# KLab/YAIK

Measured on AMD Instinct MI355X. Metric: Mpix/s tile encode (alpha reject + 7 gradient passes + 8x8 range quant), 8K RGBA, higher is better.
Workload: dtype u8/int32 (+f32 mode-selection sums)

## Files before the change

yaik_amd/csrc/yk_api.hip:

```cpp
#include "yk_common.h"
#ifdef YK_TEST_HOOKS
#include "../../include/yaik_hip_test.h"
#endif
#include <cstdio>
#include <cstring>
#include <utility>
#include <vector>

int yk_fail(yk_ctx* c, int code, const char* what, hipError_t e) {
    if (c && c->err.empty()) {
        c->err = what ? what : "error";
        if (e != hipSuccess) { c->err += ": "; c->err += hipGetErrorString(e); }
    }
    return code;
}

int yk_refuse(yk_ctx* c, int code, const char* what) {
    if (c) c->err = what ? what : "error";
    return code;
}

void yk_rebase(yk_ctx* c, int f) {
    const YkFrameStrides& fs = c->fs; auto& B = c->B;
    c->curFrame = f;
    for (int i = 0; i < 4; i++) c->plane[i] = B.plane[i] ? B.plane[i] + (size_t)f * fs.plane : nullptr;
    c->keep = B.keep + (size_t)f * fs.keep; c->bounds = B.bounds + (size_t)f * 16;
    for (int i = 0; i < 7; i++) c->bitmap[i] = B.bitmap[i] + (size_t)f * fs.bitmap[i];
    c->coverage = B.coverage + (size_t)f * fs.coverage; c->tileDef = B.tileDef + (size_t)f * fs.tileDef;
    c->tileCount = B.tileCount + (size_t)f * fs.tileCount; c->slots = B.slots + (size_t)f * fs.slots;
    c->blockSums = B.blockSums + (size_t)f * fs.blockN; c->blockCnt = B.blockCnt + (size_t)f * fs.blockN;
    c->totals = B.totals + (size_t)f * 8; c->defsOut = B.defsOut + (size_t)f * fs.defsOut; c->nibOut = B.nibOut + (size_t)f * fs.nibOut;
}

static void yk_free_image(yk_ctx* c) {
    auto F = [](auto*& p) { if (p) { (void)hipFree((void*)p); p = nullptr; } };
    auto& B = c->B;
    F(B.keep); F(B.bounds); F(c->alphaUnitBox); F(c->alphaArrive);
    F(B.small);
    for (int i = 0; i < 7; i++) B.bitmap[i] = nullptr;
    B.coverage = nullptr; B.bm0b = nullptr; B.tileInfo = nullptr; B.runSums = nullptr;
    F(B.tileDef); F(B.tileCount); F(B.slots);
    for (int i = 0; i < 3; i++) F(c->dst[i]);
    F(B.blockSums); F(B.blockCnt); F(B.totals); F(c->exportSizes); F(B.defsOut); F(B.nibOut);
    c->keep = nullptr; c->bounds = nullptr; for (int i = 0; i < 7; i++) c->bitmap[i] = nullptr;
    c->coverage = nullptr; c->tileDef = nullptr; c->tileCount = nullptr; c->slots = nullptr;
    c->blockSums = nullptr; c->blockCnt = nullptr; c->totals = nullptr; c->defsOut = nullptr; c->nibOut = nullptr;
    F(c->latticeOwner); F(c->cornerStream); F(c->cornerScratch); F(c->cornerEdgeIdx);
    F(c->preview); F(c->covCh); F(c->mapped3); F(c->ppBitmap); F(c->ppStream); F(c->ppScratch); c->ppBitmapBytes = c->ppBitmapCap = 0; c->ppStreamCap = c->ppStreamBytes = 0; c->ppScratchElems = 0;
    F(c->r1Slots); F(c->r1Params); F(c->r1Cnt); F(c->r1Pix); F(c->r1Type); c->r1Ready = false;
    F(c->pixCache); c->pixCacheValid = false;
    if (c->frameGraph) { (void)hipGraphExecDestroy(c->frameGraph); c->frameGraph = nullptr; }
    c->encoded = false; c->alphaDone = false; c->alphaFinished = false; c->cornersReady = false; c->ppActive = false; c->ppLastBit = 0; c->previewFresh = false;
}

static int yk_alloc_image(yk_ctx* c) {
    const size_t F = (size_t)c->nFrames;
    const size_t T8 = (size_t)c->tilesW * c->tilesH, MT = (size_t)c->mtW * c->mtH;
    auto& B = c->B; YkFrameStrides& fs = c->fs;
    auto up = [](size_t n, size_t a) { return (n + a - 1) / a * a; };
    fs.keep = up(MT + 4, 16);
    YK_HIP(c, hipMalloc(&B.keep, fs.keep * F + 16));
    YK_HIP(c, hipMalloc(&B.bounds, 16 * sizeof(int32_t) * F));
    {
        const size_t nUnits = (size_t)((c->fullW / 4 + 63) / 64) * c->mtH, nGroups = (nUnits + 63) / 64;
        YK_HIP(c, hipMalloc(&c->alphaUnitBox, (nUnits + nGroups) * F * 4 * sizeof(int) + 16));
        YK_HIP(c, hipMalloc(&c->alphaArrive, (nGroups + 1) * F * sizeof(uint32_t) + 16));
        YK_HIP(c, hipMemset(c->alphaArrive, 0, (nGroups + 1) * F * sizeof(uint32_t) + 16));
    }
    static const int sh[7][2] = { {4,4},{4,3},{3,4},{3,3},{3,2},{2,3},{2,2} };
    size_t cur = 0, oBm[7], oBm0b, oCov, oInfo, oRun;
    auto place = [&](size_t bytesPerFrame) { const size_t o = cur; cur = up(cur + bytesPerFrame * F + 16, 256); return o; };
    for (int i = 0; i < 7; i++) {
        const int bx = (sh[i][0] == 2) ? 32 : 64, by = (sh[i][1] == 2) ? 32 : 64;
        const size_t bits = (size_t)((c->fullW + bx - 1) / bx) * ((c->h + by - 1) / by) * ((bx >> sh[i][0]) * (by >> sh[i][1]));
        c->bitmapBytes[i] = bits >> 3;
        fs.bitmap[i] = up(c->bitmapBytes[i] + 4, 16);
        oBm[i] = place(fs.bitmap[i]);
    }
    const size_t nB64 = (size_t)((c->fullW + 63) / 64) * ((c->h + 63) / 64);
    fs.bm0b = up(nB64 * 4, 16); oBm0b = place(fs.bm0b);
    fs.coverage = up(MT, 8); oCov = place(fs.coverage * sizeof(uint16_t));
    fs.tileInfo = up(T8, 2); oInfo = place(fs.tileInfo * sizeof(uint2));
    fs.runSums = up((T8 + 7) / 8, 4); oRun = place(fs.runSums * sizeof(uint32_t));
    if (cur >= ((size_t)1 << 32)) return yk_fail(c, YK_ERR_BAD_ARG, "image too large for 32-bit offsets into the small-output arena");
    YK_HIP(c, hipMalloc(&B.small, cur));
    YK_HIP(c, hipMemset(B.small, 0, cur));
    for (int i = 0; i < 7; i++) B.bitmap[i] = B.small + oBm[i];
    B.bm0b = B.small + oBm0b; B.coverage = reinterpret_cast<uint16_t*>(B.small + oCov);
    B.tileInfo = reinterpret_cast<uint2*>(B.small + oInfo); B.runSums = reinterpret_cast<uint32_t*>(B.small + oRun);
    fs.tileDef = 3 * T8; fs.tileCount = 3 * T8; fs.slots = 3 * T8 * YK_SLOT;
    YK_HIP(c, hipMalloc(&B.tileDef, fs.tileDef * F * sizeof(uint16_t) + 16));
    YK_HIP(c, hipMalloc(&B.tileCount, fs.tileCount * F + 16));
    YK_HIP(c, hipMalloc(&B.slots, fs.slots * F + 16));
    c->nScanBlocks = (int)((T8 + 1023) / 1024);
    fs.blockN = (size_t)c->nScanBlocks * 2;
    YK_HIP(c, hipMalloc(&B.blockSums, fs.blockN * F * sizeof(uint32_t)));
    YK_HIP(c, hipMalloc(&B.blockCnt, fs.blockN * F * sizeof(uint32_t)));
    YK_HIP(c, hipMemset(B.blockCnt, 0, fs.blockN * F * sizeof(uint32_t)));
    YK_HIP(c, hipMalloc(&B.totals, 8 * sizeof(uint32_t) * F));
    fs.defsOut = 3 * T8;
// ... 75 lines not shown
int yk_create(int device, yk_ctx** out) {
    if (!out) return YK_ERR_BAD_ARG;
    *out = nullptr;
    int n = 0;
    if (hipGetDeviceCount(&n) != hipSuccess || n <= 0) return YK_ERR_NO_DEVICE;
    if (device < 0 || device >= n) return YK_ERR_BAD_ARG;
    if (hipSetDevice(device) != hipSuccess) return YK_ERR_NO_DEVICE;
    yk_ctx* c = new yk_ctx();
    c->device = device;
    if (hipDeviceGetAttribute(&c->numCU, hipDeviceAttributeMultiprocessorCount, device) != hipSuccess || c->numCU <= 0) c->numCU = 256;
    if (hipStreamCreateWithFlags(&c->ownStream, hipStreamNonBlocking) != hipSuccess) { delete c; return YK_ERR_HIP; }
    c->stream = c->ownStream;
    for (int r = 0; r < YK_EV_RING; r++) for (int i = 0; i < 5; i++) if (hipEventCreate(&c->evRing[r][i]) != hipSuccess) { delete c; return YK_ERR_HIP; }
    if (yk_qtab_get(c) != YK_OK) { yk_destroy(c); return YK_ERR_HIP; }
    *out = c;
    return YK_OK;
}

void yk_destroy(yk_ctx* c) {
    if (!c) return;
    (void)hipSetDevice(c->device);
    (void)hipStreamSynchronize(c->stream);
    yk_free_image(c);
    yk_lut_destroy(c);
    yk_lut_dec_destroy(c);
    auto F = [](auto*& p) { if (p) { (void)hipFree((void*)p); p = nullptr; } };
    yk_dec_free(c);
    F(c->ownedPlanes); F(c->pxStage); F(c->dScratch); F(c->dAlpha); F(c->dAvScratch); F(c->avState); F(c->avPay); F(c->av6);
    for (int r = 0; r < YK_EV_RING; r++) for (int i = 0; i < 5; i++) if (c->evRing[r][i]) (void)hipEventDestroy(c->evRing[r][i]);
    for (int st = 0; st < YK_NUM_STAGES; st++) for (int k = 0; k < YK_STAGE_RING; k++) for (int i = 0; i < 2; i++) if (c->stEv[st][k][i]) (void)hipEventDestroy(c->stEv[st][k][i]);
    if (c->frameGraph) (void)hipGraphExecDestroy(c->frameGraph);
    if (c->evHandoff) (void)hipEventDestroy(c->evHandoff);
    if (c->evPixCopy) (void)hipEventDestroy(c->evPixCopy);
    if (c->evFusedAfter) (void)hipEventDestroy(c->evFusedAfter);
    if (c->auxStream) (void)hipStreamDestroy(c->auxStream);
    if (c->ownStream) (void)hipStreamDestroy(c->ownStream);
    delete c;
}

const char* yk_last_error(const yk_ctx* c) { return c ? c->err.c_str() : "null handle"; }

int yk_set_stream(yk_ctx* c, void* s) {
    if (!c) return YK_ERR_BAD_ARG;
    hipStream_t next = s ? (hipStream_t)s : c->ownStream;
    if (next == c->stream) return YK_OK;
    YK_HIP(c, hipSetDevice(c->device));
    if (!c->evHandoff) YK_HIP(c, hipEventCreateWithFlags(&c->evHandoff, hipEventDisableTiming));
    if (hipEventRecord(c->evHandoff, c->stream) == hipSuccess) YK_HIP(c, hipStreamWaitEvent(next, c->evHandoff, 0));
    else (void)hipGetLastError();
    c->stream = next;
    return YK_OK;
}

int yk_synchronize(yk_ctx* c) {
    if (!c) return YK_ERR_BAD_ARG;
    YK_HIP(c, hipSetDevice(c->device));
    YK_HIP(c, hipStreamSynchronize(c->stream));
    return YK_OK;
}

int yk_set_image(yk_ctx* c, int fullW, int fullH, int nPlanes, int y0, int h, int haloRows) {
    if (!c) return YK_ERR_BAD_ARG;
    if (fullW < 8 || fullH < 8 || (fullW & 7) || (fullH & 7) || fullW > 32760 || fullH > 32760) return yk_fail(c, YK_ERR_BAD_ARG, "image size must be a multiple of 8 and fit s16 fields");
    if (nPlanes != 3 && nPlanes != 4) return yk_fail(c, YK_ERR_BAD_ARG, "nPlanes must be 3 or 4");
    if (y0 < 0 || h < 8 || (h & 7) || y0 + h > fullH || (y0 & 63)) return yk_fail(c, YK_ERR_BAD_ARG, "stripe rows must start on a multiple of 64 and lie inside the image");
    if (y0 + h < fullH && ((h & 63) || haloRows != 1)) return yk_fail(c, YK_ERR_BAD_ARG, "inner stripes need h % 64 == 0 and one halo row");
    if (y0 + h == fullH && haloRows != 0) return yk_fail(c, YK_ERR_BAD_ARG, "the last stripe has no halo row");
    YK_HIP(c, hipSetDevice(c->device));
// ... 328 lines not shown
    YK_HIP(c, hipSetDevice(c->device));
    if (wantDst) {
        const size_t n = (size_t)c->fullW * c->h;
        for (int p = 0; p < 3; p++) {
            if (!c->dst[p]) YK_HIP(c, hipMalloc(&c->dst[p], n * sizeof(int32_t)));
            if (c->dstFill == 0 || c->dstFill == -1) YK_HIP(c, hipMemsetAsync(c->dst[p], c->dstFill & 255, n * sizeof(int32_t), c->stream));
            else {
                std::vector<int32_t> f(n, c->dstFill);
                YK_HIP(c, hipMemcpyAsync(c->dst[p], f.data(), n * sizeof(int32_t), hipMemcpyHostToDevice, c->stream));
                YK_HIP(c, hipStreamSynchronize(c->stream));
            }
        }
    }
    hipEvent_t* ev = c->evRing[c->evHead % YK_EV_RING];
    if (!c->evAlphaInCur) { YK_HIP(c, hipEventRecord(ev[0], c->stream)); YK_HIP(c, hipEventRecord(ev[1], c->stream)); }
    if (c->fusedAfter) { YK_HIP(c, hipStreamWaitEvent(c->stream, c->fusedAfter, 0)); c->fusedAfter = nullptr; }
    YK_HIP(c, hipEventRecord(ev[2], c->stream));
    int rc = yk_launch_encode(c, rejectFactor, mode3BitOnly, wantDst); if (rc) return rc;
    YK_HIP(c, hipEventRecord(ev[3], c->stream));
    rc = yk_launch_pack(c); if (rc) return rc;
    YK_HIP(c, hipEventRecord(ev[4], c->stream));
    c->evAlphaInCur = false;
    c->evHead++;
    if (c->evHead - c->evTail > YK_EV_RING) c->evTail = c->evHead - YK_EV_RING;
    c->encoded = true; c->dstValid = wantDst != 0; c->cornersReady = false; c->ppActive = false; c->ppLastBit = 0; c->previewFresh = false; c->nextCornerPass = 0; c->r1Ready = false;
    return YK_OK;
}

int yk_order_fused_after(yk_ctx* c, const yk_ctx* other) {
    if (!c || !other) return YK_ERR_BAD_ARG;
    if (c->device != other->device) return yk_fail(c, YK_ERR_BAD_ARG, "yk_order_fused_after: handles of one device");
    c->fusedAfter = nullptr;
    if (!other->evHead) return YK_OK;
    YK_HIP(c, hipSetDevice(c->device));
    if (!c->auxStream) YK_HIP(c, hipStreamCreateWithFlags(&c->auxStream, hipStreamNonBlocking));
    if (!c->evFusedAfter) YK_HIP(c, hipEventCreateWithFlags(&c->evFusedAfter, hipEventDisableTiming));
    static const int afterPack = getenv("YK_ORDER_AFTER_PACK") ? atoi(getenv("YK_ORDER_AFTER_PACK")) : 0;
    YK_HIP(c, hipStreamWaitEvent(c->auxStream, other->evRing[(other->evHead - 1) % YK_EV_RING][afterPack ? 4 : 3], 0));
    YK_HIP(c, hipEventRecord(c->evFusedAfter, c->auxStream));
    c->fusedAfter = c->evFusedAfter;
    return YK_OK;
}

int yk_encode_batch(yk_ctx* c, int rejectFactor, int mode3BitOnly) {
    if (!c) return YK_ERR_BAD_ARG;
    if (!c->B.plane[0]) return yk_fail(c, YK_ERR_STATE, "bind planes first");
    if (rejectFactor < 0 || rejectFactor > 64) return yk_fail(c, YK_ERR_BAD_ARG, "rejectFactor out of range");
    if (c->y0 != 0 || c->h != c->fullH) return yk_fail(c, YK_ERR_STATE, "batches hold whole images");
    if (c->kernelVersion != 2) return yk_fail(c, YK_ERR_STATE, "batches need kernel version 2");
    if (c->nFrames > 1 && c->fs.plane == 0) return yk_fail(c, YK_ERR_STATE, "yk_bind_device_batch first");
    YK_HIP(c, hipSetDevice(c->device));
    hipEvent_t* ev = c->evRing[c->evHead % YK_EV_RING];
    YK_HIP(c, hipEventRecord(ev[0], c->stream));
    int rc = YK_OK;
    if (c->nPlanes == 4) rc = yk_launch_alpha(c, true);
    if (rc) return rc;
    YK_HIP(c, hipEventRecord(ev[1], c->stream));
    if (c->fusedAfter) { YK_HIP(c, hipStreamWaitEvent(c->stream, c->fusedAfter, 0)); c->fusedAfter = nullptr; }
    YK_HIP(c, hipEventRecord(ev[2], c->stream));
    rc = yk_launch_encode(c, rejectFactor, mode3BitOnly, 0, true); if (rc) return rc;
    YK_HIP(c, hipEventRecord(ev[3], c->stream));
    rc = yk_launch_pack(c, true); if (rc) return rc;
    YK_HIP(c, hipEventRecord(ev[4], c->stream));
    c->evAlphaInCur = false; c->evHead++;
    if (c->evHead - c->evTail > YK_EV_RING) c->evTail = c->evHead - YK_EV_RING;
    c->alphaDone = c->nPlanes == 4; c->alphaFinished = true;
    c->encoded = true; c->dstValid = false; c->cornersReady = false; c->ppActive = false; c->ppLastBit = 0; c->previewFresh = false; c->nextCornerPass = 0; c->r1Ready = false;
    return YK_OK;
}

int yk_encode_frame(yk_ctx* c, int rejectFactor, int mode3BitOnly) {
    if (!c) return YK_ERR_BAD_ARG;
    if (!c->plane[0]) return yk_fail(c, YK_ERR_STATE, "bind planes first");
// ... 239 lines not shown
```

yaik_amd/csrc/yk_common.h:

```cpp
#pragma once
#include <hip/hip_runtime.h>
#include <stdint.h>
#include <stddef.h>
#include <string>
#include "../../include/yaik_hip.h"

#define YK_BLK      64
#define YK_LSTRIDE  68
#define YK_LROWS    65
#define YK_EV_RING  64
#define YK_SLOT     32
#define YK_NUM_STAGES 8
#define YK_STAGE_RING 16

struct YkFrameStrides {
    unsigned long long plane, keep, bitmap[7], coverage, tileDef, tileCount, slots, blockN, defsOut, nibOut;
    unsigned long long bm0b, tileInfo, runSums;
};

struct YkEncodeParams {
    const int32_t* plane[4];
    int strideElems;
    int w, h;
    int hAvail;
// ... 14 lines not shown
    int xBB64, yBB64, xBB32, yBB32;
    int nFrames;
    const uint8_t* qtab;
    uint8_t* small;
    uint32_t oBm[7], oBm0b, oCov, oInfo, oRun;
    uint4* pixCache;
    YkFrameStrides fs;
};

struct yk_ctx {
    int device = -1;
    int numCU = 256;
    const uint8_t* qtab = nullptr;
    hipStream_t ownStream = nullptr;
    hipStream_t stream = nullptr;
    std::string err;
    int fullW = 0, fullH = 0, nPlanes = 0, y0 = 0, h = 0, halo = 0;
    int tilesW = 0, tilesH = 0, mtW = 0, mtH = 0;
    int nFrames = 1, curFrame = 0;
    YkFrameStrides fs = {};
    struct Bases {
        const int32_t* plane[4]; uint8_t* keep; int32_t* bounds; uint8_t* bitmap[7]; uint16_t* coverage; uint16_t* tileDef; uint8_t* tileCount;
        uint8_t* slots; uint32_t* blockSums; uint32_t* blockCnt; uint32_t* totals; uint16_t* defsOut; uint8_t* nibOut;
        uint8_t* small;
        uint8_t* bm0b; uint2* tileInfo; uint32_t* runSums;
    } B = {};
    const int32_t* plane[4] = {nullptr, nullptr, nullptr, nullptr};
    int strideElems = 0;
    int32_t* ownedPlanes = nullptr; size_t ownedPlanesBytes = 0;
    uint8_t* pxStage = nullptr; size_t pxStageBytes = 0;
    hipEvent_t evPixCopy = nullptr;
    uint8_t* keep = nullptr;
    int32_t* bounds = nullptr;
    int* alphaUnitBox = nullptr;
    uint32_t* alphaArrive = nullptr;
    int boundsOff = 8;
    bool alphaDone = false, alphaFinished = false;
    int32_t hostBounds[4] = {0, 0, 0, 0}; int hostDiscard = 1, hostHasChunk = 0;
    uint8_t* bitmap[7] = {}; size_t bitmapBytes[7] = {};
    uint16_t* coverage = nullptr;
    uint16_t* tileDef = nullptr; uint8_t* tileCount = nullptr; uint8_t* slots = nullptr;
    int32_t* dst[3] = {nullptr, nullptr, nullptr}; int32_t dstFill = -1; bool dstValid = false;
    uint32_t* blockSums = nullptr;
    uint32_t* blockCnt = nullptr;
    uint32_t* totals = nullptr;
    unsigned long long* exportSizes = nullptr;
    hipEvent_t evHandoff = nullptr;
    hipEvent_t fusedAfter = nullptr;
    hipEvent_t evFusedAfter = nullptr; hipStream_t auxStream = nullptr;
    uint16_t* defsOut = nullptr;
    uint8_t*  nibOut = nullptr;
    size_t nibStride = 0;
    int nScanBlocks = 0;
    bool encoded = false;
    uint32_t* latticeOwner = nullptr; size_t latticeElems = 0;
    uint8_t* cornerStream = nullptr; size_t cornerCap = 0;
    uint32_t* cornerScratch = nullptr; size_t cornerScratchElems = 0;
    uint32_t* cornerEdgeIdx = nullptr;
    bool cornersReady = false; int nextCornerPass = 0;
    size_t cornerOff[7] = {}, cornerBytes[7] = {};
    const uint32_t* cornerTotalsDev = nullptr; bool cornerTotalsPending = false;
    const uint32_t* r1TotalsDev = nullptr; bool r1TotalsPending = false;
    uint16_t* covCh = nullptr; size_t covChStride = 0;
    uint8_t* mapped3 = nullptr;
    uint32_t* ppBitmap = nullptr; size_t ppBitmapBytes = 0; uint8_t* ppStream = nullptr; size_t ppStreamCap = 0, ppStreamBytes = 0;
    uint32_t* ppScratch = nullptr; size_t ppScratchElems = 0, ppBitmapCap = 0; int ppAccepted = 0; bool ppActive = false;
    int ppLastBit = 0, ppLastSx = 0, ppLastSy = 0;
    int32_t* preview = nullptr; bool previewFresh = false;
    struct YkLutState* lut = nullptr;
    struct YkLutDecState* lutDec = nullptr;
    uint8_t* r1Slots = nullptr; uint8_t* r1Params = nullptr; uint32_t* r1Cnt = nullptr; uint8_t* r1Pix = nullptr; uint8_t* r1Type = nullptr;
    uint32_t r1Tiles = 0, r1PixCount = 0; bool r1Ready = false;
    uint4* pixCache = nullptr; bool pixCacheOn = false, pixCacheValid = false;
    uint32_t r1EndTiles[3] = {}, r1EndPix[3] = {};
    int dw = 0, dh = 0; uint8_t* dPlanes = nullptr; size_t dPlaneSize = 0;
    uint8_t* dMapRGB = nullptr; uint32_t* dLatticeOwner = nullptr; uint8_t* dTile4 = nullptr; size_t dTile4Size = 0;
    uint8_t* dScratch = nullptr; size_t dScratchBytes = 0;
    uint8_t* dLoaded = nullptr;
    bool dSplit = false;
    uint8_t* dAlpha = nullptr; size_t dAlphaBytes = 0; bool dAlphaValid = false;
    uint8_t* dAvScratch = nullptr; size_t dAvScratchBytes = 0;
    int32_t* avState = nullptr; uint8_t* avPay = nullptr; size_t avPayCap = 0;
// ... 44 lines not shown
```

yaik_amd/csrc/yk_stages.hip:

```cpp
#include "yk_common.h"
#ifdef YK_TEST_HOOKS
#include "../../include/yaik_hip_test.h"
#endif
#include "yk_device.h"

typedef int yk_i4 __attribute__((ext_vector_type(4)));
#ifndef YK_ALPHA_INFLIGHT
#define YK_ALPHA_INFLIGHT 8
#endif
#ifndef YK_ALPHA_THREADS
#define YK_ALPHA_THREADS 256
#endif
#define YK_ALPHA_WAVES (YK_ALPHA_THREADS / 64)
#ifndef YK_ALPHA_ROWS
#define YK_ALPHA_ROWS 2
#endif
__global__ __launch_bounds__(YK_ALPHA_THREADS) void yk_alpha_kernel(const int32_t* __restrict__ alpha0, int strideElems, int w, int h, int y0,
                                                       uint8_t* __restrict__ keep0, int mtW, int mtH, int32_t* __restrict__ bounds,
                                                       int nFrames, unsigned long long planeStride, unsigned long long keepStride,
                                                       int* __restrict__ unitBox0, uint32_t* __restrict__ arrive0) {
    __shared__ int s_box[YK_ALPHA_WAVES][4];
    const int lane = threadIdx.x & 63, wv = threadIdx.x >> 6;
    const int vecPerRow = w >> 2;
    const int nSeg = (vecPerRow + YK_ALPHA_THREADS - 1) / YK_ALPHA_THREADS;
    const int nRowUnits = (mtH + YK_ALPHA_ROWS - 1) / YK_ALPHA_ROWS;
    const int nUnits = nSeg * nRowUnits, nGroups = (nUnits + 63) >> 6;
    for (long long uu = blockIdx.x; uu < (long long)nUnits * nFrames; uu += gridDim.x) {
        const int f = (int)(uu / nUnits), u = (int)(uu - (long long)f * nUnits);
        const int32_t* alpha = alpha0 + (size_t)f * planeStride;
        uint8_t* keep = keep0 + (size_t)f * keepStride;
        int* unitBox = unitBox0 + (size_t)f * (nUnits + nGroups) * 4;
        uint32_t* arrive = arrive0 + (size_t)f * (nGroups + 1);
        const int tyU = u / nSeg, seg = u - tyU * nSeg;
        const int xv = seg * YK_ALPHA_THREADS + (int)threadIdx.x;
        const bool inX = xv < vecPerRow;
        const bool tileLane = (lane & 3) == 0;
        const int tx = xv >> 2;
        int colLo = 0x7FFFFFFF, colHi = -1, rowLo = 0x7FFFFFFF, rowHi = -1;
#pragma unroll
        for (int r = 0; r < YK_ALPHA_ROWS; r++) {
            const int ty = tyU * YK_ALPHA_ROWS + r;
            if (ty >= mtH) break;
            const int32_t* col = alpha + (size_t)(ty * 16) * strideElems + (size_t)xv * 4;
            int nz = 0;
#pragma unroll
            for (int kb = 0; kb < 16 / YK_ALPHA_INFLIGHT; kb++) {
                yk_i4 a[YK_ALPHA_INFLIGHT];
#pragma unroll
                for (int k = 0; k < YK_ALPHA_INFLIGHT; k++) {
                    const int y = ty * 16 + kb * YK_ALPHA_INFLIGHT + k;
                    a[k] = (yk_i4){0, 0, 0, 0};
                    if (inX && y < h) a[k] = __builtin_nontemporal_load(reinterpret_cast<const yk_i4*>(col + (size_t)(kb * YK_ALPHA_INFLIGHT + k) * strideElems));
                }
#pragma unroll
                for (int k = 0; k < YK_ALPHA_INFLIGHT; k++) nz |= a[k].x | a[k].y | a[k].z | a[k].w;
            }
            const unsigned long long b = __ballot(nz != 0);
            const bool kept = ((b >> (lane & ~3)) & 0xFULL) != 0;
            if (tileLane && tx < mtW) keep[(size_t)ty * mtW + tx] = kept ? 1 : 0;
            const unsigned long long kb64 = __ballot(tileLane && kept && tx < mtW);
            if (kb64) {
                const int t0 = seg * (YK_ALPHA_THREADS / 4) + wv * 16;
                colLo = min(colLo, t0 + ((__ffsll((long long)kb64) - 1) >> 2));
                colHi = max(colHi, t0 + ((63 - __clzll((long long)kb64)) >> 2));
                rowLo = min(rowLo, ty); rowHi = max(rowHi, ty);
            }
        }
        if (lane == 0) { s_box[wv][0] = colLo; s_box[wv][1] = colHi; s_box[wv][2] = rowLo; s_box[wv][3] = rowHi; }
        __syncthreads();
        if (wv == 0) {
            unsigned long long* ub = reinterpret_cast<unsigned long long*>(unitBox);
            auto putBox = [&](const int slot, const int bx0, const int by0, const int bx1, const int by1) {
                __hip_atomic_store(&ub[slot * 2], ((unsigned long long)(uint32_t)by0 << 32) | (uint32_t)bx0, __ATOMIC_RELAXED, __HIP_MEMORY_SCOPE_AGENT);
                __hip_atomic_store(&ub[slot * 2 + 1], ((unsigned long long)(uint32_t)by1 << 32) | (uint32_t)bx1, __ATOMIC_RELAXED, __HIP_MEMORY_SCOPE_AGENT);
                __builtin_amdgcn_s_waitcnt(0);
            };
            auto foldBoxes = [&](const int first, const int n, int& x0, int& gy0, int& x1, int& gy1) {
                x0 = 9999999; gy0 = 9999999; x1 = -1; gy1 = -1;
                for (int k = lane; k < n; k += 64) {
                    const unsigned long long a = __hip_atomic_load(&ub[(first + k) * 2], __ATOMIC_RELAXED, __HIP_MEMORY_SCOPE_AGENT);
                    const unsigned long long bb = __hip_atomic_load(&ub[(first + k) * 2 + 1], __ATOMIC_RELAXED, __HIP_MEMORY_SCOPE_AGENT);
                    x0 = min(x0, (int)(uint32_t)a); gy0 = min(gy0, (int)(uint32_t)(a >> 32)); x1 = max(x1, (int)(uint32_t)bb); gy1 = max(gy1, (int)(uint32_t)(bb >> 32));
                }
#pragma unroll
                for (int d = 1; d < 64; d <<= 1) {
                    x0 = min(x0, __shfl_xor(x0, d)); x1 = max(x1, __shfl_xor(x1, d));
                    gy0 = min(gy0, __shfl_xor(gy0, d)); gy1 = max(gy1, __shfl_xor(gy1, d));
                }
            };
            const int g = u >> 6, inGroup = min(64, nUnits - (g << 6));
            uint32_t lastOfGroup = 0;
            if (lane == 0) {
                int lo = s_box[0][0], hi = s_box[0][1], rlo = s_box[0][2], rhi = s_box[0][3];
#pragma unroll
                for (int k = 1; k < YK_ALPHA_WAVES; k++) { lo = min(lo, s_box[k][0]); hi = max(hi, s_box[k][1]); rlo = min(rlo, s_box[k][2]); rhi = max(rhi, s_box[k][3]); }
                const bool any = hi >= 0;
                putBox(u, any ? lo * 16 : 9999999, any ? y0 + rlo * 16 : 9999999, any ? hi * 16 + 16 : -1, any ? y0 + rhi * 16 + 16 : -1);
                lastOfGroup = __hip_atomic_fetch_add(&arrive[g], 1u, __ATOMIC_RELAXED, __HIP_MEMORY_SCOPE_AGENT) == (uint32_t)inGroup - 1u ? 1u : 0u;
            }
            if (__builtin_amdgcn_readfirstlane((int)lastOfGroup)) {
                int x0, gy0, x1, gy1;
                foldBoxes(g << 6, inGroup, x0, gy0, x1, gy1);
                uint32_t lastOfFrame = 0;
                if (lane == 0) {
                    putBox(nUnits + g, x0, gy0, x1, gy1);
                    arrive[g] = 0u;
                    lastOfFrame = __hip_atomic_fetch_add(&arrive[nGroups], 1u, __ATOMIC_RELAXED, __HIP_MEMORY_SCOPE_AGENT) == (uint32_t)nGroups - 1u ? 1u : 0u;
                }
                if (__builtin_amdgcn_readfirstlane((int)lastOfFrame)) {
                    foldBoxes(nUnits, nGroups, x0, gy0, x1, gy1);
                    if (lane == 0) { int32_t* acc = bounds + (size_t)f * 16 + 8; acc[0] = x0; acc[1] = gy0; acc[2] = x1; acc[3] = gy1; arrive[nGroups] = 0u; }
                }
            }
        }
        if (uu + gridDim.x < (long long)nUnits * nFrames) __syncthreads();
    }
}

__global__ void yk_alpha_publish_kernel(int32_t* __restrict__ bounds, int srcOff, int fullW, int fullH) {
    bounds += (size_t)blockIdx.x * 16;
    const int b0 = bounds[srcOff], b1 = bounds[srcOff + 1], b2 = bounds[srcOff + 2], b3 = bounds[srcOff + 3];
    bounds[0] = b0; bounds[1] = b1; bounds[2] = b2; bounds[3] = b3;
    bounds[4] = (b0 == 0 && b1 == 0 && b2 == fullW && b3 == fullH) ? 1 : 0;
}

#define YK_SCAN_TILE 1024

__global__ __launch_bounds__(1024) void yk_scan1_kernel(const uint8_t* __restrict__ tileCount, size_t T8, uint32_t* __restrict__ blockCnt) {
    __shared__ uint32_t s_tmp[32];
    const size_t i = (size_t)blockIdx.x * YK_SCAN_TILE + threadIdx.x;
    const uint32_t c = (i < T8) ? tileCount[i] : 0;
    uint32_t tot2, totN;
    yk_block_exscan(c ? 1u : 0u, s_tmp, &tot2);
    yk_block_exscan(c, s_tmp, &totN);
    if (threadIdx.x == 0) { blockCnt[(size_t)blockIdx.x * 2] = totN; blockCnt[(size_t)blockIdx.x * 2 + 1] = tot2; }
}

__device__ __forceinline__ void yk_scan2_body(uint32_t* __restrict__ blockCnt, uint32_t* __restrict__ blockSums, int nBlocks, uint32_t* __restrict__ totals, uint32_t* s_tmp) {
    uint32_t baseN = 0, baseD = 0;
    for (int start = 0; start < nBlocks; start += 1024) {
        const int i = start + threadIdx.x;
        const uint32_t n = i < nBlocks ? blockCnt[i * 2] : 0, d = i < nBlocks ? blockCnt[i * 2 + 1] : 0;
        uint32_t totN, totD;
        const uint32_t en = yk_block_exscan(n, s_tmp, &totN);
        const uint32_t ed = yk_block_exscan(d, s_tmp, &totD);
        if (i < nBlocks) {
            blockSums[i * 2] = baseN + en; blockSums[i * 2 + 1] = baseD + ed;
            blockCnt[i * 2] = 0; blockCnt[i * 2 + 1] = 0;
// ... 78 lines not shown
        const uint32_t ed = yk_block_exscan(c ? 1u : 0u, s_tmp, &totD);
        const uint32_t baseN = blockCnt ? preN : blockSums[(size_t)blockIdx.x * 2], baseD = blockCnt ? preD : blockSums[(size_t)blockIdx.x * 2 + 1];
        s_off[threadIdx.x] = (baseN + en) >> 1;
        s_cnt[threadIdx.x] = (uint8_t)c;
        if (c) {
            defsOut[baseD + ed] = (uint16_t)d01; defsOut[T8 + baseD + ed] = (uint16_t)(d01 >> 16); defsOut[2 * T8 + baseD + ed] = (uint16_t)d2;
        }
    }
    __syncthreads();
    const int piece = threadIdx.x & 3;
#pragma unroll
    for (int p = 0; p < 3; p++) {
        uint8_t* out = reinterpret_cast<uint8_t*>(nibOut + (size_t)p * nibStrideWords);
#pragma unroll
        for (int it = 0; it < 4; it++) {
            const int t = it * 256 + (threadIdx.x >> 2);
            const size_t i = i0 + t;
            if (i < T8 && piece * 8 < (s_cnt[t] >> 1))
                *reinterpret_cast<uint2*>(out + s_off[t] + piece * 8) = *reinterpret_cast<const uint2*>(slots + ((size_t)p * T8 + i) * YK_SLOT + piece * 8);
        }
    }
}

static int (*g_crossCheckLauncher)(hipStream_t, const YkEncodeParams*) = nullptr;
#ifdef YK_TEST_HOOKS
extern "C" int yk_set_cross_check_launcher(void* fn) { g_crossCheckLauncher = reinterpret_cast<int (*)(hipStream_t, const YkEncodeParams*)>(fn); return YK_OK; }
#endif

int yk_launch_alpha(yk_ctx* c, bool batch) {
    const int F = batch ? c->nFrames : 1;
    uint8_t* keep = batch ? c->B.keep : c->keep;
    int32_t* bounds = batch ? c->B.bounds : c->bounds;
    const int32_t* alpha = batch ? c->B.plane[3] : c->plane[3];
    const int nSeg = (c->fullW / 4 + YK_ALPHA_THREADS - 1) / YK_ALPHA_THREADS;
    const long long nUnits = (long long)nSeg * ((c->mtH + YK_ALPHA_ROWS - 1) / YK_ALPHA_ROWS) * F;
    const long long maxWG = 4096LL * (256 / YK_ALPHA_THREADS);
    hipLaunchKernelGGL(yk_alpha_kernel, dim3((unsigned)(nUnits < maxWG ? nUnits : maxWG)), dim3(YK_ALPHA_THREADS), 0, c->stream, alpha, c->strideElems, c->fullW, c->h, c->y0,
                       keep, c->mtW, c->mtH, bounds, F, (unsigned long long)c->fs.plane, (unsigned long long)c->fs.keep, c->alphaUnitBox, c->alphaArrive);
    YK_HIP(c, hipGetLastError());
    c->boundsOff = 8;
    return YK_OK;
}

int yk_launch_alpha_finish(yk_ctx* c, const int32_t* globalBBox) {
    if (globalBBox) {
        int32_t b[5] = { globalBBox[0], globalBBox[1], globalBBox[2], globalBBox[3], 0 };
        b[4] = (b[0] == 0 && b[1] == 0 && b[2] == c->fullW && b[3] == c->fullH) ? 1 : 0;
        YK_HIP(c, hipMemcpyAsync(c->bounds, b, sizeof b, hipMemcpyHostToDevice, c->stream));
        c->boundsOff = 0;
    }
    return YK_OK;
}

int yk_launch_encode(yk_ctx* c, int rejectFactor, int mode3BitOnly, int wantDst, bool batch) {
    YkEncodeParams P;
    for (int i = 0; i < 4; i++) P.plane[i] = batch ? c->B.plane[i] : c->plane[i];
    P.strideElems = c->strideElems; P.w = c->fullW; P.h = c->h; P.hAvail = c->h + c->halo; P.y0 = c->y0; P.fullH = c->fullH;
    P.rejectFactor = rejectFactor; P.startMode = mode3BitOnly ? 3 : 0; P.wantDst = wantDst; P.ablate = c->ablate;
    P.keep = (c->nPlanes == 4) ? (batch ? c->B.keep : c->keep) : nullptr;
    P.bounds = (c->nPlanes == 4) ? (batch ? c->B.bounds : c->bounds) + c->boundsOff : nullptr;
    for (int i = 0; i < 7; i++) P.bitmap[i] = batch ? c->B.bitmap[i] : c->bitmap[i];
    P.coverage = batch ? c->B.coverage : c->coverage; P.tileDef = batch ? c->B.tileDef : c->tileDef;
    P.tileCount = batch ? c->B.tileCount : c->tileCount; P.slots = batch ? c->B.slots : c->slots;
    P.blockCnt = c->kernelVersion == 2 ? (batch ? c->B.blockCnt : c->blockCnt) : nullptr;
    for (int i = 0; i < 3; i++) P.dst[i] = c->dst[i];
    P.tilesW = c->tilesW; P.tilesH = c->tilesH; P.mtW = c->mtW; P.mtH = c->mtH;
    P.xBB64 = (c->fullW + 63) / 64; P.yBB64 = (c->h + 63) / 64; P.xBB32 = (c->fullW + 31) / 32; P.yBB32 = (c->h + 31) / 32;
    P.nFrames = batch ? c->nFrames : 1; P.fs = c->fs;
    P.qtab = c->qtab;
    P.small = c->B.small;
    for (int i = 0; i < 7; i++) P.oBm[i] = (uint32_t)(c->B.bitmap[i] - c->B.small);
// ... 111 lines not shown
```

yaik_amd/encoder.py:

```python
from __future__ import annotations

import ctypes as C
from typing import NamedTuple

import numpy as np

from ._lib import YaikError, lib

PASSES = [(4, 4), (4, 3), (3, 4), (3, 3), (3, 2), (2, 3), (2, 2)]


_HANDLE_LIB: dict = {}


def _chk(h, rc: int, L=None):
    if rc != 0:
        owner = L or _HANDLE_LIB.get(getattr(h, "value", h)) or lib()
        msg = owner.yk_last_error(h)
        raise YaikError(f"yaik_hip error {rc}: {msg.decode() if msg else '?'}")


class PixelLayout(NamedTuple):
    frames: int
    rows: int
# ... 164 lines not shown
        self._keepalive = pixels

    def validate_planes(self) -> int:
        n = C.c_size_t(0)
        _chk(self._h, self._L.yk_validate_planes(self._h, C.byref(n)))
        return int(n.value)

    def alpha_reject(self):
        _chk(self._h, self._L.yk_alpha_reject(self._h))

    def stripe_bbox(self) -> np.ndarray:
        b = np.zeros(4, dtype=np.int32)
        _chk(self._h, self._L.yk_get_stripe_bbox(self._h, b.ctypes.data))
        return b

    def alpha_finish(self, global_bbox: np.ndarray | None = None):
        if global_bbox is None:
            _chk(self._h, self._L.yk_alpha_finish(self._h, None))
        else:
            g = np.ascontiguousarray(global_bbox, dtype=np.int32)
            _chk(self._h, self._L.yk_alpha_finish(self._h, g.ctypes.data))

    def mip_prefilter(self) -> dict:
        if self.n == 4:
            self.alpha_reject()
            self.alpha_finish(None)
        return self.alpha_result()

    def alpha_result(self) -> dict:
        L = self._L
        b = np.zeros(4, dtype=np.int32); tb = np.zeros(4, dtype=np.int32)
        has, rem = C.c_int(), C.c_int()
        _chk(self._h, L.yk_alpha_result(self._h, b.ctypes.data, C.byref(has), C.byref(rem), tb.ctypes.data))
        out = np.zeros(max(1, (self.w // 16) * (self.full_h // 16) // 8 + 8), dtype=np.uint8)
        nb = C.c_size_t()
        _chk(self._h, L.yk_alpha_bitmap(self._h, out.ctypes.data, out.size, C.byref(nb)))
        return {"has_chunk": bool(has.value), "bounds": b, "remaining": rem.value, "tile_bbox": tb, "bitmap": out[:nb.value].copy()}

    def alpha_values(self, force8bit: bool = True) -> dict | None:

        class _Info(C.Structure):
            _fields_ = [("mode", C.c_int32), ("bbox", C.c_int32 * 4), ("rawSize", C.c_uint32)]

        info, n = _Info(), C.c_size_t()
        out = np.empty(self.w * self.full_h, dtype=np.uint8)
        _chk(self._h, self._L.yk_alpha_values(self._h, int(force8bit), C.byref(info), out.ctypes.data, out.size, C.byref(n)))
        if info.mode < 0:
            return None
        return {"mode": int(info.mode), "bbox": tuple(int(v) for v in info.bbox), "payload": out[:n.value].copy()}

    def encode(self, reject_factor: int = 3, mode3bit_only: bool = False, want_dst: bool = False, dst_fill: int = -1):
        L = self._L
        _chk(self._h, L.yk_set_dst_fill(self._h, dst_fill))
        _chk(self._h, L.yk_encode_tiles(self._h, reject_factor, int(mode3bit_only), int(want_dst)))

    def set_batch(self, frames):
        import torch
        L = self._L
        assert frames.dtype == torch.int32 and frames.is_cuda and frames.is_contiguous() and frames.dim() == 4
        F, n, h, w = frames.shape
        self.n, self.h, self.w, self.full_h, self.y0, self.frames = n, h, w, h, 0, F
        _chk(self._h, L.yk_set_image(self._h, w, h, n, 0, h, 0))
        _chk(self._h, L.yk_set_batch(self._h, F))
        torch.cuda.current_stream(frames.device).synchronize()
        base = frames.data_ptr()
        ptrs = (C.c_void_p * 4)(*[base + i * h * w * 4 if i < n else None for i in range(4)])
        _chk(self._h, L.yk_bind_device_batch(self._h, ptrs, w, n * h * w))
# ... 186 lines not shown
```

Before: 213,500.

## Split alpha reject into streaming kernel plus separate bbox fold kernel

Replaces the persistent alpha-reject kernel, which used atomic arrival counters and last-block folding, with a 3D-grid kernel of one wave per 64-vector segment. Each wave handles 32 rows, issuing 16 loads in flight per batch, and writes a packed 32-bit keep-mask record per unit. A second single-wave-per-frame kernel ORs these records to compute the bounding box. This removes atomics, shared-memory and barrier synchronisation, and the group-arrival scheme, at the cost of an extra launch. It also drops the aux-stream event hop in fused ordering and makes a minor Python bitmap-size fix.

After: 203,500. 4.7% lower.

```diff
diff --git a/yaik_amd/csrc/yk_api.hip b/yaik_amd/csrc/yk_api.hip
--- a/yaik_amd/csrc/yk_api.hip
+++ b/yaik_amd/csrc/yk_api.hip
@@ -35,7 +35,7 @@
 static void yk_free_image(yk_ctx* c) {
     auto F = [](auto*& p) { if (p) { (void)hipFree((void*)p); p = nullptr; } };
     auto& B = c->B;
-    F(B.keep); F(B.bounds); F(c->alphaUnitBox); F(c->alphaArrive);
+    F(B.keep); F(B.bounds); F(c->alphaUnitBox);
     F(B.small);
     for (int i = 0; i < 7; i++) B.bitmap[i] = nullptr;
     B.coverage = nullptr; B.bm0b = nullptr; B.tileInfo = nullptr; B.runSums = nullptr;
@@ -62,10 +62,11 @@
     YK_HIP(c, hipMalloc(&B.keep, fs.keep * F + 16));
     YK_HIP(c, hipMalloc(&B.bounds, 16 * sizeof(int32_t) * F));
     {
-        const size_t nUnits = (size_t)((c->fullW / 4 + 63) / 64) * c->mtH, nGroups = (nUnits + 63) / 64;
-        YK_HIP(c, hipMalloc(&c->alphaUnitBox, (nUnits + nGroups) * F * 4 * sizeof(int) + 16));
-        YK_HIP(c, hipMalloc(&c->alphaArrive, (nGroups + 1) * F * sizeof(uint32_t) + 16));
-        YK_HIP(c, hipMemset(c->alphaArrive, 0, (nGroups + 1) * F * sizeof(uint32_t) + 16));
+        const int nSeg = (c->fullW / 4 + 63) / 64;
+        c->alphaSegPitch = 4; while (c->alphaSegPitch < nSeg) c->alphaSegPitch <<= 1;
+        const size_t bytes = (size_t)((c->mtH + 1) / 2) * c->alphaSegPitch * F * sizeof(uint32_t);
+        YK_HIP(c, hipMalloc(&c->alphaUnitBox, bytes));
+        YK_HIP(c, hipMemset(c->alphaUnitBox, 0, bytes));
     }
     static const int sh[7][2] = { {4,4},{4,3},{3,4},{3,3},{3,2},{2,3},{2,2} };
     size_t cur = 0, oBm[7], oBm0b, oCov, oInfo, oRun;
@@ -207,8 +208,6 @@
     if (c->frameGraph) (void)hipGraphExecDestroy(c->frameGraph);
     if (c->evHandoff) (void)hipEventDestroy(c->evHandoff);
     if (c->evPixCopy) (void)hipEventDestroy(c->evPixCopy);
-    if (c->evFusedAfter) (void)hipEventDestroy(c->evFusedAfter);
-    if (c->auxStream) (void)hipStreamDestroy(c->auxStream);
     if (c->ownStream) (void)hipStreamDestroy(c->ownStream);
     delete c;
 }
@@ -603,13 +602,7 @@
     if (c->device != other->device) return yk_fail(c, YK_ERR_BAD_ARG, "yk_order_fused_after: handles of one device");
     c->fusedAfter = nullptr;
     if (!other->evHead) return YK_OK;
-    YK_HIP(c, hipSetDevice(c->device));
-    if (!c->auxStream) YK_HIP(c, hipStreamCreateWithFlags(&c->auxStream, hipStreamNonBlocking));
-    if (!c->evFusedAfter) YK_HIP(c, hipEventCreateWithFlags(&c->evFusedAfter, hipEventDisableTiming));
-    static const int afterPack = getenv("YK_ORDER_AFTER_PACK") ? atoi(getenv("YK_ORDER_AFTER_PACK")) : 0;
-    YK_HIP(c, hipStreamWaitEvent(c->auxStream, other->evRing[(other->evHead - 1) % YK_EV_RING][afterPack ? 4 : 3], 0));
-    YK_HIP(c, hipEventRecord(c->evFusedAfter, c->auxStream));
-    c->fusedAfter = c->evFusedAfter;
+    c->fusedAfter = other->evRing[(other->evHead - 1) % YK_EV_RING][3];
     return YK_OK;
 }
 
diff --git a/yaik_amd/csrc/yk_common.h b/yaik_amd/csrc/yk_common.h
--- a/yaik_amd/csrc/yk_common.h
+++ b/yaik_amd/csrc/yk_common.h
@@ -70,8 +70,8 @@
     hipEvent_t evPixCopy = nullptr;
     uint8_t* keep = nullptr;
     int32_t* bounds = nullptr;
-    int* alphaUnitBox = nullptr;
-    uint32_t* alphaArrive = nullptr;
+    uint32_t* alphaUnitBox = nullptr;
+    int alphaSegPitch = 0;
     int boundsOff = 8;
     bool alphaDone = false, alphaFinished = false;
     int32_t hostBounds[4] = {0, 0, 0, 0}; int hostDiscard = 1, hostHasChunk = 0;
@@ -85,7 +85,6 @@
     unsigned long long* exportSizes = nullptr;
     hipEvent_t evHandoff = nullptr;
     hipEvent_t fusedAfter = nullptr;
-    hipEvent_t evFusedAfter = nullptr; hipStream_t auxStream = nullptr;
     uint16_t* defsOut = nullptr;
     uint8_t*  nibOut = nullptr;
     size_t nibStride = 0;
diff --git a/yaik_amd/csrc/yk_stages.hip b/yaik_amd/csrc/yk_stages.hip
--- a/yaik_amd/csrc/yk_stages.hip
+++ b/yaik_amd/csrc/yk_stages.hip
@@ -5,115 +5,94 @@
 #include "yk_device.h"
 
 typedef int yk_i4 __attribute__((ext_vector_type(4)));
-#ifndef YK_ALPHA_INFLIGHT
-#define YK_ALPHA_INFLIGHT 8
-#endif
-#ifndef YK_ALPHA_THREADS
-#define YK_ALPHA_THREADS 256
-#endif
-#define YK_ALPHA_WAVES (YK_ALPHA_THREADS / 64)
-#ifndef YK_ALPHA_ROWS
-#define YK_ALPHA_ROWS 2
-#endif
-__global__ __launch_bounds__(YK_ALPHA_THREADS) void yk_alpha_kernel(const int32_t* __restrict__ alpha0, int strideElems, int w, int h, int y0,
-                                                       uint8_t* __restrict__ keep0, int mtW, int mtH, int32_t* __restrict__ bounds,
-                                                       int nFrames, unsigned long long planeStride, unsigned long long keepStride,
-                                                       int* __restrict__ unitBox0, uint32_t* __restrict__ arrive0) {
-    __shared__ int s_box[YK_ALPHA_WAVES][4];
-    const int lane = threadIdx.x & 63, wv = threadIdx.x >> 6;
+#define YK_ALPHA_DEPTH 16
+template <int K0, int N> __device__ __forceinline__ void yk_alpha_batch(const char*& row, int& y, const int h, const size_t pitch, const uint32_t laneOff, int (&nz)[2]) {
+    yk_i4 a[N];
+#pragma unroll
+    for (int k = 0; k < N; k++) {
+        a[k] = __builtin_nontemporal_load(reinterpret_cast<const yk_i4*>(row + laneOff));
+        if (++y < h) row += pitch;
+    }
+    static_assert(N == 16, "one operand per load of the batch");
+#define YK_A4(i) "+v"(a[i]), "+v"(a[i + 1]), "+v"(a[i + 2]), "+v"(a[i + 3])
+    asm volatile("" : YK_A4(0), YK_A4(4), YK_A4(8), YK_A4(12));
+#undef YK_A4
+#pragma unroll
+    for (int k = 0; k < N; k++) nz[(K0 + k) >> 4] |= a[k].x | a[k].y | a[k].z | a[k].w;
+}
+
+__global__ __launch_bounds__(64) __attribute__((amdgpu_waves_per_eu(4, 4)))
+void yk_alpha_kernel(const int32_t* __restrict__ alpha0, int strideElems, int w, int h, uint8_t* __restrict__ keep0, int mtW, int mtH,
+                     unsigned long long planeStride, unsigned long long keepStride, uint32_t* __restrict__ unitBox0, int segPitch) {
+    const int lane = threadIdx.x, seg = blockIdx.x, tyU = blockIdx.y;
+    const size_t f = blockIdx.z;
     const int vecPerRow = w >> 2;
-    const int nSeg = (vecPerRow + YK_ALPHA_THREADS - 1) / YK_ALPHA_THREADS;
-    const int nRowUnits = (mtH + YK_ALPHA_ROWS - 1) / YK_ALPHA_ROWS;
-    const int nUnits = nSeg * nRowUnits, nGroups = (nUnits + 63) >> 6;
-    for (long long uu = blockIdx.x; uu < (long long)nUnits * nFrames; uu += gridDim.x) {
-        const int f = (int)(uu / nUnits), u = (int)(uu - (long long)f * nUnits);
-        const int32_t* alpha = alpha0 + (size_t)f * planeStride;
-        uint8_t* keep = keep0 + (size_t)f * keepStride;
-        int* unitBox = unitBox0 + (size_t)f * (nUnits + nGroups) * 4;
-        uint32_t* arrive = arrive0 + (size_t)f * (nGroups + 1);
-        const int tyU = u / nSeg, seg = u - tyU * nSeg;
-        const int xv = seg * YK_ALPHA_THREADS + (int)threadIdx.x;
-        const bool inX = xv < vecPerRow;
-        const bool tileLane = (lane & 3) == 0;
-        const int tx = xv >> 2;
-        int colLo = 0x7FFFFFFF, colHi = -1, rowLo = 0x7FFFFFFF, rowHi = -1;
-#pragma unroll
-        for (int r = 0; r < YK_ALPHA_ROWS; r++) {
-            const int ty = tyU * YK_ALPHA_ROWS + r;
-            if (ty >= mtH) break;
-            const int32_t* col = alpha + (size_t)(ty * 16) * strideElems + (size_t)xv * 4;
-            int nz = 0;
-#pragma unroll
-            for (int kb = 0; kb < 16 / YK_ALPHA_INFLIGHT; kb++) {
-                yk_i4 a[YK_ALPHA_INFLIGHT];
-#pragma unroll
-                for (int k = 0; k < YK_ALPHA_INFLIGHT; k++) {
-                    const int y = ty * 16 + kb * YK_ALPHA_INFLIGHT + k;
-                    a[k] = (yk_i4){0, 0, 0, 0};
-                    if (inX && y < h) a[k] = __builtin_nontemporal_load(reinterpret_cast<const yk_i4*>(col + (size_t)(kb * YK_ALPHA_INFLIGHT + k) * strideElems));
-                }
-#pragma unroll
-                for (int k = 0; k < YK_ALPHA_INFLIGHT; k++) nz |= a[k].x | a[k].y | a[k].z | a[k].w;
+    const int xv = seg * 64 + lane;
+    const bool inX = xv < vecPerRow;
+    uint32_t laneOff = (uint32_t)min(xv, vecPerRow - 1) * 16u;
+    const size_t pitch = (size_t)strideElems * 4;
+    int y = tyU * 32;
+    const char* row = reinterpret_cast<const char*>(alpha0 + f * planeStride) + (size_t)y * pitch;
+    int nz[2] = {0, 0};
+    yk_alpha_batch<0, YK_ALPHA_DEPTH>(row, y, h, pitch, laneOff, nz);
+    asm volatile("" : "+v"(laneOff) : "v"(nz[0]), "v"(nz[1]));
+    yk_alpha_batch<YK_ALPHA_DEPTH, 32 - YK_ALPHA_DEPTH>(row, y, h, pitch, laneOff, nz);
+    uint8_t* keep = keep0 + f * keepStride;
+    const int tx = xv >> 2;
+    uint32_t rec = 0;
+#pragma unroll
+    for (int r = 0; r < 2; r++) {
+        const int ty = tyU * 2 + r;
+        if (ty >= mtH) break;
+        unsigned long long m = __ballot(inX && nz[r] != 0);
+        m |= m >> 1; m |= m >> 2; m &= 0x1111111111111111ULL;
+        if ((lane & 3) == 0 && tx < mtW) keep[(size_t)ty * mtW + tx] = (uint8_t)((m >> lane) & 1ULL);
+        m = (m | (m >> 3)) & 0x0303030303030303ULL; m = (m | (m >> 6)) & 0x000F000F000F000FULL;
+        m = (m | (m >> 12)) & 0x000000FF000000FFULL; m = (m | (m >> 24)) & 0xFFFFULL;
+        rec |= (uint32_t)m << (16 * r);
+    }
+    if (lane == 0) unitBox0[(f * gridDim.y + tyU) * segPitch + seg] = rec;
+}
+
+__global__ __launch_bounds__(64) __attribute__((amdgpu_waves_per_eu(4)))
+void yk_alpha_fold_kernel(const uint32_t* __restrict__ unitBox0, int segPitch, int nRowUnits, int y0, int32_t* __restrict__ bounds) {
+    const int lane = threadIdx.x;
+    const size_t f = blockIdx.x;
+    const int n4 = (nRowUnits * segPitch) >> 2, lg = __ffs(segPitch) - 1;
+    const uint4* rec = reinterpret_cast<const uint4*>(unitBox0 + f * nRowUnits * segPitch);
+    uint32_t c[4] = {0u, 0u, 0u, 0u};
+    int rowLo = 0x7FFFFFFF, rowHi = -1;
+    for (int i0 = 0; i0 < n4; i0 += 64 * 16) {
+        uint4 v[16];
+#pragma unroll
+        for (int k = 0; k < 16; k++) { const int i = i0 + k * 64 + lane; v[k] = i < n4 ? rec[i] : make_uint4(0u, 0u, 0u, 0u); }
+#pragma unroll
+        for (int k = 0; k < 16; k++) {
+            c[0] |= v[k].x; c[1] |= v[k].y; c[2] |= v[k].z; c[3] |= v[k].w;
+            const uint32_t o = v[k].x | v[k].y | v[k].z | v[k].w;
+            if (o) {
+                const int tyU = ((i0 + k * 64 + lane) << 2) >> lg;
+                rowLo = min(rowLo, tyU * 2 + ((o & 0xFFFFu) ? 0 : 1)); rowHi = max(rowHi, tyU * 2 + ((o >> 16) ? 1 : 0));
             }
-            const unsigned long long b = __ballot(nz != 0);
-            const bool kept = ((b >> (lane & ~3)) & 0xFULL) != 0;
-            if (tileLane && tx < mtW) keep[(size_t)ty * mtW + tx] = kept ? 1 : 0;
-            const unsigned long long kb64 = __ballot(tileLane && kept && tx < mtW);
-            if (kb64) {
-                const int t0 = seg * (YK_ALPHA_THREADS / 4) + wv * 16;
-                colLo = min(colLo, t0 + ((__ffsll((long long)kb64) - 1) >> 2));
-                colHi = max(colHi, t0 + ((63 - __clzll((long long)kb64)) >> 2));
-                rowLo = min(rowLo, ty); rowHi = max(rowHi, ty);
-            }
-        }
-        if (lane == 0) { s_box[wv][0] = colLo; s_box[wv][1] = colHi; s_box[wv][2] = rowLo; s_box[wv][3] = rowHi; }
-        __syncthreads();
-        if (wv == 0) {
-            unsigned long long* ub = reinterpret_cast<unsigned long long*>(unitBox);
-            auto putBox = [&](const int slot, const int bx0, const int by0, const int bx1, const int by1) {
-                __hip_atomic_store(&ub[slot * 2], ((unsigned long long)(uint32_t)by0 << 32) | (uint32_t)bx0, __ATOMIC_RELAXED, __HIP_MEMORY_SCOPE_AGENT);
-                __hip_atomic_store(&ub[slot * 2 + 1], ((unsigned long long)(uint32_t)by1 << 32) | (uint32_t)bx1, __ATOMIC_RELAXED, __HIP_MEMORY_SCOPE_AGENT);
-                __builtin_amdgcn_s_waitcnt(0);
-            };
-            auto foldBoxes = [&](const int first, const int n, int& x0, int& gy0, int& x1, int& gy1) {
-                x0 = 9999999; gy0 = 9999999; x1 = -1; gy1 = -1;
-                for (int k = lane; k < n; k += 64) {
-                    const unsigned long long a = __hip_atomic_load(&ub[(first + k) * 2], __ATOMIC_RELAXED, __HIP_MEMORY_SCOPE_AGENT);
-                    const unsigned long long bb = __hip_atomic_load(&ub[(first + k) * 2 + 1], __ATOMIC_RELAXED, __HIP_MEMORY_SCOPE_AGENT);
-                    x0 = min(x0, (int)(uint32_t)a); gy0 = min(gy0, (int)(uint32_t)(a >> 32)); x1 = max(x1, (int)(uint32_t)bb); gy1 = max(gy1, (int)(uint32_t)(bb >> 32));
-                }
-#pragma unroll
-                for (int d = 1; d < 64; d <<= 1) {
-                    x0 = min(x0, __shfl_xor(x0, d)); x1 = max(x1, __shfl_xor(x1, d));
-                    gy0 = min(gy0, __shfl_xor(gy0, d)); gy1 = max(gy1, __shfl_xor(gy1, d));
-                }
-            };
-            const int g = u >> 6, inGroup = min(64, nUnits - (g << 6));
-            uint32_t lastOfGroup = 0;
-            if (lane == 0) {
-                int lo = s_box[0][0], hi = s_box[0][1], rlo = s_box[0][2], rhi = s_box[0][3];
-#pragma unroll
-                for (int k = 1; k < YK_ALPHA_WAVES; k++) { lo = min(lo, s_box[k][0]); hi = max(hi, s_box[k][1]); rlo = min(rlo, s_box[k][2]); rhi = max(rhi, s_box[k][3]); }
-                const bool any = hi >= 0;
-                putBox(u, any ? lo * 16 : 9999999, any ? y0 + rlo * 16 : 9999999, any ? hi * 16 + 16 : -1, any ? y0 + rhi * 16 + 16 : -1);
-                lastOfGroup = __hip_atomic_fetch_add(&arrive[g], 1u, __ATOMIC_RELAXED, __HIP_MEMORY_SCOPE_AGENT) == (uint32_t)inGroup - 1u ? 1u : 0u;
-            }
-            if (__builtin_amdgcn_readfirstlane((int)lastOfGroup)) {
-                int x0, gy0, x1, gy1;
-                foldBoxes(g << 6, inGroup, x0, gy0, x1, gy1);
-                uint32_t lastOfFrame = 0;
-                if (lane == 0) {
-                    putBox(nUnits + g, x0, gy0, x1, gy1);
-                    arrive[g] = 0u;
-                    lastOfFrame = __hip_atomic_fetch_add(&arrive[nGroups], 1u, __ATOMIC_RELAXED, __HIP_MEMORY_SCOPE_AGENT) == (uint32_t)nGroups - 1u ? 1u : 0u;
-                }
-                if (__builtin_amdgcn_readfirstlane((int)lastOfFrame)) {
-                    foldBoxes(nUnits, nGroups, x0, gy0, x1, gy1);
-                    if (lane == 0) { int32_t* acc = bounds + (size_t)f * 16 + 8; acc[0] = x0; acc[1] = gy0; acc[2] = x1; acc[3] = gy1; arrive[nGroups] = 0u; }
-                }
-            }
-        }
-        if (uu + gridDim.x < (long long)nUnits * nFrames) __syncthreads();
+        }
+    }
+    int colLo = 0x7FFFFFFF, colHi = -1;
+#pragma unroll
+    for (int j = 0; j < 4; j++) {
+        const uint32_t m = (c[j] | (c[j] >> 16)) & 0xFFFFu;
+        const int t0 = ((((lane << 2) & (segPitch - 1)) + j) << 4);
+        if (m) { colLo = min(colLo, t0 + __ffs((int)m) - 1); colHi = max(colHi, t0 + 31 - __clz((int)m)); }
+    }
+#pragma unroll
+    for (int d = 1; d < 64; d <<= 1) {
+        colLo = min(colLo, __shfl_xor(colLo, d)); colHi = max(colHi, __shfl_xor(colHi, d));
+        rowLo = min(rowLo, __shfl_xor(rowLo, d)); rowHi = max(rowHi, __shfl_xor(rowHi, d));
+    }
+    if (lane == 0) {
+        const bool any = colHi >= 0;
+        int32_t* acc = bounds + f * 16 + 8;
+        acc[0] = any ? colLo * 16 : 9999999; acc[1] = any ? y0 + rowLo * 16 : 9999999;
+        acc[2] = any ? colHi * 16 + 16 : -1; acc[3] = any ? y0 + rowHi * 16 + 16 : -1;
     }
 }
 
@@ -258,11 +237,10 @@
     uint8_t* keep = batch ? c->B.keep : c->keep;
     int32_t* bounds = batch ? c->B.bounds : c->bounds;
     const int32_t* alpha = batch ? c->B.plane[3] : c->plane[3];
-    const int nSeg = (c->fullW / 4 + YK_ALPHA_THREADS - 1) / YK_ALPHA_THREADS;
-    const long long nUnits = (long long)nSeg * ((c->mtH + YK_ALPHA_ROWS - 1) / YK_ALPHA_ROWS) * F;
-    const long long maxWG = 4096LL * (256 / YK_ALPHA_THREADS);
-    hipLaunchKernelGGL(yk_alpha_kernel, dim3((unsigned)(nUnits < maxWG ? nUnits : maxWG)), dim3(YK_ALPHA_THREADS), 0, c->stream, alpha, c->strideElems, c->fullW, c->h, c->y0,
-                       keep, c->mtW, c->mtH, bounds, F, (unsigned long long)c->fs.plane, (unsigned long long)c->fs.keep, c->alphaUnitBox, c->alphaArrive);
+    const int nSeg = (c->fullW / 4 + 63) / 64, nRowUnits = (c->mtH + 1) / 2;
+    hipLaunchKernelGGL(yk_alpha_kernel, dim3((unsigned)nSeg, (unsigned)nRowUnits, (unsigned)F), dim3(64), 0, c->stream, alpha, c->strideElems, c->fullW, c->h,
+                       keep, c->mtW, c->mtH, (unsigned long long)c->fs.plane, (unsigned long long)c->fs.keep, c->alphaUnitBox, c->alphaSegPitch);
+    hipLaunchKernelGGL(yk_alpha_fold_kernel, dim3((unsigned)F), dim3(64), 0, c->stream, c->alphaUnitBox, c->alphaSegPitch, nRowUnits, c->y0, bounds);
     YK_HIP(c, hipGetLastError());
     c->boundsOff = 8;
     return YK_OK;
diff --git a/yaik_amd/encoder.py b/yaik_amd/encoder.py
--- a/yaik_amd/encoder.py
+++ b/yaik_amd/encoder.py
@@ -220,7 +220,7 @@
         b = np.zeros(4, dtype=np.int32); tb = np.zeros(4, dtype=np.int32)
         has, rem = C.c_int(), C.c_int()
         _chk(self._h, L.yk_alpha_result(self._h, b.ctypes.data, C.byref(has), C.byref(rem), tb.ctypes.data))
-        out = np.zeros(max(1, (self.w // 16) * (self.full_h // 16) // 8 + 8), dtype=np.uint8)
+        out = np.zeros(((self.w + 15) // 16) * ((self.full_h + 15) // 16) // 8 + 8, dtype=np.uint8)
         nb = C.c_size_t()
         _chk(self._h, L.yk_alpha_bitmap(self._h, out.ctypes.data, out.size, C.byref(nb)))
         return {"has_chunk": bool(has.value), "bounds": b, "remaining": rem.value, "tile_bbox": tb, "bitmap": out[:nb.value].copy()}
```
